# blairstar/NaturalDiffusion

Hardware: AMD Instinct MI355X
Metric: images/sec at 15-step Natural Inference (CIFAR10 32x32, NCSN++), 3-stream throughput (higher is better)
Workload: dtype bf16; 1 GPU; CIFAR10 NI 15-step step_15_weight_173.npz B=512/GPU NCSN++ 61.8M bf16, ni_step fp64 history; nfe=15, batch_per_gpu=512, streams=3

## Files before the change

### include/natinf_ncsnpp.h

```cpp
#ifndef NATINF_NCSNPP_H
#define NATINF_NCSNPP_H

#include <stdint.h>
#include "natinf.h"

#ifdef __cplusplus
extern "C" {
#endif

typedef struct natinf_ncsnpp* natinf_ncsnpp_t;

#define NATINF_NCSNPP_KEEP_ACTIVATIONS 1
#define NATINF_NCSNPP_DDPM 2

int64_t natinf_ncsnpp_param_count(void);
int64_t natinf_ncsnpp_packed_bytes(void);
int64_t natinf_ncsnpp_handle_param_count(natinf_ncsnpp_t h);
int64_t natinf_ncsnpp_handle_packed_bytes(natinf_ncsnpp_t h);
int64_t natinf_ncsnpp_workspace_bytes(natinf_ncsnpp_t h, int max_batch);

int natinf_ncsnpp_create(natinf_ncsnpp_t* out, int flags);
int natinf_ncsnpp_destroy(natinf_ncsnpp_t h);

int natinf_ncsnpp_describe(natinf_ncsnpp_t h, char* buf, int cap);
// ... 19 lines not shown
int natinf_debug_gemm_fp8(int M, int N, int K, const void* a8, const float* a_scale, const void* a_mx, const void* b8, const float* b_scale,
                          const float* bias_n, void* c, void* c_mx, int c_mode, int iters, natinf_stream_t stream);
int natinf_debug_conv_gn_up(int flags);
int natinf_debug_conv_gn_fin(float* fin_scale, float* fin_shift, const float* gamma, const float* beta, int channels_per_group, float mul);
int natinf_debug_conv_gn(int res, int B, int N, int cin, int c1, const void* x, const float* scale, const float* shift, const void* w_packed, void* w_frag,
                         const void* a1, const float* bias_n, const void* resid, float out_scale, void* out, float* gn_part, int iters,
                         natinf_stream_t stream);
#define NATINF_ATTN_BLOCK_OFF_WQKV 0
#define NATINF_ATTN_BLOCK_OFF_W3 393216
#define NATINF_ATTN_BLOCK_OFF_FOLD_WQK 524288
#define NATINF_ATTN_BLOCK_OFF_FOLD_WVO 786432
#define NATINF_ATTN_BLOCK_OFF_FOLD_CQ 1048576
#define NATINF_ATTN_BLOCK_OFF_FOLD_BO 1049600
#define NATINF_ATTN_BLOCK_OFF_WQK_PACKED 1050624
#define NATINF_ATTN_BLOCK_OFF_WVO_PACKED 1181696
#define NATINF_ATTN_BLOCK_PACKED_BYTES 1312768
#define NATINF_ATTN_BLOCK_SCRATCH_BYTES_PER_SAMPLE 393216
int natinf_debug_attn_block(int plan, int B, const void* x, int x_ld, const float* scale, const float* shift, const float* w, const float* bias,
                            void* packed, void* scratch, void* out, int o_ld, float out_scale, float* gn_part, natinf_stream_t stream);
int natinf_set_gemm_variant(int variant);
int natinf_set_gemm_epilogue(int fp32_slab);
int natinf_set_gemm_pref512(int on);
int natinf_set_gemm_half_issue(int on);
int natinf_set_gemm_round_model(int on);
int natinf_set_gemm_w128(int on);
int natinf_set_gemm_raster(int rows);
int natinf_set_fuse_gn(int on);
int natinf_set_conv_gn_wide(int mask);
int natinf_set_conv_gn_w128(int mask);
int natinf_set_conv_gn_w128_min_k(int shape, int k);
int natinf_set_conv_gn_regw(int on);
int natinf_set_fuse_up(int on);
int natinf_set_fuse_up_fold(int on);
int natinf_debug_fold_up_weights(const float* w, int N, int cin, float w_mul, float* out_f32, void* out_packed, natinf_stream_t stream);
int natinf_debug_conv_up_fold(int B, int N, int cin, const void* x, const float* scale, const float* shift, const float* w, void* w_packed, void* h_scratch,
                              const float* bias_n, const float* rowvec, float out_scale, void* out, float* gn_part, int iters, natinf_stream_t stream);
int natinf_set_fuse_head(int on);
int natinf_set_fuse_gn8(int on);
int natinf_set_fuse_gn4(int on);
int natinf_set_fuse_fin(int on);
int natinf_set_conv_gn_warm(int mask);
int natinf_set_attn256(int on);
int natinf_set_attn_proj(int on);
int natinf_set_attn_waves8(int on);
int natinf_set_attn_block(int on);
int natinf_set_attn_qkv(int on);
int natinf_set_conv_gn8_tile(int one_image);
int natinf_set_gemm_splitk(int on);
int natinf_debug_set_splitk_workspace(float* ws, int max_slices);
int natinf_debug_timestamps(void* dev_buf16);

int natinf_ncsnpp_profile(natinf_ncsnpp_t h, int enable);
int natinf_ncsnpp_profile_read(natinf_ncsnpp_t h, double* ms_by_class , int64_t* launches_by_class );

int natinf_gemm_profile(int enable);
int natinf_gemm_profile_read(char* buf, int cap);

int natinf_ncsnpp_debug_tap(natinf_ncsnpp_t h, int module_idx, float* out, int64_t capacity_elems,
                            natinf_stream_t stream);

int natinf_debug_gn_stats(const void* x, int ld, int C, int HW, int B, const float* gamma, const float* beta, float* scale, float* shift, float eps, float out_mul,
                          natinf_stream_t stream);
int natinf_debug_gn_finalize(const float* P0, int tps0, int quads0, const float* P1, int tps1, int quads1, int C, int HW, int B, const float* gamma, const float* beta,
                             float* scale, float* shift, float eps, float out_mul, natinf_stream_t stream);
int natinf_debug_gn_fold(const float* P, int tps, int quads, int fold, int B, float* out, natinf_stream_t stream);
int natinf_debug_gn_apply(const void* x, int ld, int C, int logW, int logHW, int B, const float* scale, const float* shift, void* y, void* xr, int act, int mode, int pad,
// ... 13 lines not shown
```

### naturaldiffusion_amd/_lib.py

```python
from __future__ import annotations

import ctypes as C
import os
from pathlib import Path

os.environ.setdefault("GPU_MAX_HW_QUEUES", "8")

_HERE = Path(__file__).resolve().parent
LIB_PATH = Path(os.environ.get("NATINF_LIB", _HERE / "libnatinf.so"))

if not LIB_PATH.exists():
    raise ImportError(
        f"{LIB_PATH} not found: build it with `make -C {_HERE / 'csrc'}` "
        "(or `python -c 'import __graft_entry__ as g; g.build()'`). "
        "naturaldiffusion_amd has no CPU or eager-PyTorch fallback.")

lib = C.CDLL(str(LIB_PATH))

_p, _i32, _i64, _f32, _f64 = C.c_void_p, C.c_int, C.c_int64, C.c_float, C.c_double

SIGNATURES = {
    "natinf_abi_version": (C.c_int, []),
    "natinf_strerror": (C.c_char_p, [_i32]),
    "natinf_probe": (C.c_int, []),
# ... 38 lines not shown
    "natinf_weighted_mean_f16": (C.c_int, [_p, _p, _p, _p, _i32, _f32, _i64, _p]),
    "natinf_flow_input_f16": (C.c_int, [_p, _p, _p, _f32, _f32, _i64, _p]),
    "natinf_ncsnpp_param_count": (C.c_int64, []),
    "natinf_ncsnpp_workspace_bytes": (C.c_int64, [_p, _i32]),
    "natinf_ncsnpp_packed_bytes": (C.c_int64, []),
    "natinf_ncsnpp_handle_param_count": (_i64, [_p]),
    "natinf_ncsnpp_handle_packed_bytes": (_i64, [_p]),
    "natinf_ncsnpp_create": (C.c_int, [C.POINTER(_p), _i32]),
    "natinf_ncsnpp_describe": (C.c_int, [_p, C.c_char_p, _i32]),
    "natinf_ncsnpp_destroy": (C.c_int, [_p]),
    "natinf_ncsnpp_load": (C.c_int, [_p, _p, _i64, _p, _i64, _p]),
    "natinf_ncsnpp_share": (C.c_int, [_p, _p]),
    "natinf_ncsnpp_forward": (C.c_int, [_p, _p, _p, _p, _i32, _p, _i64, _p]),
    "natinf_ncsnpp_debug_tap": (C.c_int, [_p, _i32, _p, _i64, _p]),
    "natinf_ncsnpp_describe_gemms": (C.c_int, [_p, _i32, C.c_char_p, _i32]),
    "natinf_debug_gemm": (C.c_int, [_i32, _i32, _i32, _i32, _i32, _i32, _i32, _i32, _p, _p, _p, _p, _p, _i32, _f32, _i32, _p]),
    "natinf_set_gemm_variant": (C.c_int, [_i32]),
    "natinf_debug_timestamps": (C.c_int, [_p]),
    "natinf_set_gemm_epilogue": (C.c_int, [_i32]),
    "natinf_debug_gemm_fused": (C.c_int, [_i32, _i32, _i32, _i32, _p, _p, _p, _p, _p, _p, _i32, _p, _p, _f32, _i32, _p, _i32, _p, _p, _i32, _p]),
    "natinf_set_gemm_pref512": (C.c_int, [_i32]),
    "natinf_set_gemm_half_issue": (C.c_int, [_i32]),
    "natinf_set_gemm_raster": (C.c_int, [_i32]),
    "natinf_set_gemm_round_model": (C.c_int, [_i32]),
    "natinf_set_gemm_w128": (C.c_int, [_i32]),
    "natinf_set_fuse_gn": (C.c_int, [_i32]),
    "natinf_set_conv_gn_wide": (C.c_int, [_i32]),
    "natinf_set_attn_block": (C.c_int, [_i32]),
    "natinf_set_conv_gn_w128": (C.c_int, [_i32]),
    "natinf_set_conv_gn_w128_min_k": (C.c_int, [_i32, _i32]),
    "natinf_set_conv_gn_regw": (C.c_int, [_i32]),
    "natinf_set_fuse_up": (C.c_int, [_i32]),
    "natinf_set_fuse_up_fold": (C.c_int, [_i32]),
    "natinf_debug_fold_up_weights": (C.c_int, [_p, _i32, _i32, _f32, _p, _p, _p]),
    "natinf_debug_conv_up_fold": (C.c_int, [_i32, _i32, _i32, _p, _p, _p, _p, _p, _p, _p, _p, _f32, _p, _p, _i32, _p]),
    "natinf_set_fuse_head": (C.c_int, [_i32]),
    "natinf_set_fuse_gn8": (C.c_int, [_i32]),
    "natinf_set_fuse_gn4": (C.c_int, [_i32]),
    "natinf_set_fuse_fin": (C.c_int, [_i32]),
    "natinf_set_attn_proj": (C.c_int, [_i32]),
    "natinf_set_attn_waves8": (C.c_int, [_i32]),
    "natinf_set_attn_qkv": (C.c_int, [_i32]),
    "natinf_set_conv_gn_warm": (C.c_int, [_i32]),
    "natinf_set_attn256": (C.c_int, [_i32]),
    "natinf_set_conv_gn8_tile": (C.c_int, [_i32]),
    "natinf_set_gemm_splitk": (C.c_int, [_i32]),
    "natinf_debug_set_splitk_workspace": (C.c_int, [_p, _i32]),
    "natinf_debug_set_conv_operand": (C.c_int, [_i32, _p, _i32]),
    "natinf_debug_conv_gn": (C.c_int, [_i32, _i32, _i32, _i32, _i32, _p, _p, _p, _p, _p, _p, _p, _p, _f32, _p, _p, _i32, _p]),
    "natinf_debug_conv_gn_up": (C.c_int, [_i32]),
    "natinf_debug_conv_gn_fin": (C.c_int, [_p, _p, _p, _p, _i32, _f32]),
    "natinf_debug_attn_block": (C.c_int, [_i32, _i32, _p, _i32, _p, _p, _p, _p, _p, _p, _p, _i32, _f32, _p, _p]),
    "natinf_debug_gn_stats": (C.c_int, [_p, _i32, _i32, _i32, _i32, _p, _p, _p, _p, _f32, _f32, _p]),
    "natinf_debug_gn_finalize": (C.c_int, [_p, _i32, _i32, _p, _i32, _i32, _i32, _i32, _i32, _p, _p, _p, _p, _f32, _f32, _p]),
    "natinf_debug_gn_fold": (C.c_int, [_p, _i32, _i32, _i32, _i32, _p, _p]),
    "natinf_debug_gn_apply": (C.c_int, [_p, _i32, _i32, _i32, _i32, _i32, _p, _p, _p, _p, _i32, _i32, _i32, _p]),
    "natinf_debug_head_conv": (C.c_int, [_p, _i32, _i32, _p, _p, _p, _p, _p, _p]),
    "natinf_debug_time_embed": (C.c_int, [_p, _p, _i32, _p]),
    "natinf_debug_stem_im2col": (C.c_int, [_p, _p, _i32, _p]),
    "natinf_debug_pack_conv": (C.c_int, [_p, _p, _i32, _i32, _i32, _i32, _i32, _i32, _i32, _f32, _p]),
    "natinf_debug_pack_transpose": (C.c_int, [_p, _p, _i32, _i32, _i32, _p]),
    "natinf_debug_nhwc_to_nchw": (C.c_int, [_p, _i32, _i32, _i32, _i32, _p, _p]),
    "natinf_ncsnpp_profile": (C.c_int, [_p, _i32]),
    "natinf_ncsnpp_profile_read": (C.c_int, [_p, C.POINTER(C.c_double), C.POINTER(C.c_int64)]),
    "natinf_debug_quant_fp8_rows": (C.c_int, [_p, _p, _p, _i32, _i32, _p]),
    "natinf_debug_gemm_fp8": (C.c_int, [_i32, _i32, _i32, _p, _p, _p, _p, _p, _p, _p, _p, _i32, _i32, _p]),
# ... 156 lines not shown
```

### naturaldiffusion_amd/csrc/gemm_dma.h

```cpp
#pragma once
#include "ncsnpp_kernels.h"

#ifndef NATINF_SETPRIO
#define NATINF_SETPRIO 0
#endif

namespace ncsn {

template <int WM, int WN, int TM, int TN, int AVAIL>
struct EpiCfg {
    static constexpr int CROW = WN * TN * 16 + 4;
    static constexpr int bytes(int rb) { return WM * rb * 16 * CROW * 4; }
    static constexpr int RB = bytes(TM) <= AVAIL ? TM : (bytes(TM / 2) <= AVAIL ? TM / 2 : (bytes(TM / 4) <= AVAIL ? TM / 4 : 1));
    static constexpr int SLAB_ROWS = WM * RB * 16;
    static constexpr int SLAB_BYTES = bytes(RB);
    static_assert(TM % RB == 0 && SLAB_BYTES <= AVAIL, "epilogue staging does not fit");
    static constexpr int PROW = WN * TN * 16 * 2 + 16;
    static constexpr int PACK_SLAB = WM * TM * 16 * PROW;
    static constexpr int PACK_BYTES = PACK_SLAB + WM * WN * TN * 4 * 8;
    static constexpr bool PACK_OK = PACK_BYTES <= AVAIL;
    static constexpr int NEED = PACK_OK && PACK_BYTES > SLAB_BYTES ? PACK_BYTES : SLAB_BYTES;
};

template <int WM, int WN, int TM, int TN>
struct DmaCfg {
    static constexpr int NW = WM * WN, THREADS = NW * 64;
    static constexpr int BM_ = WM * TM * 16, BN_ = WN * TN * 16;
    static constexpr int STAGE_BYTES = (BM_ + BN_) * BK * 2;
    static constexpr int PA = BM_ / 8 / NW, PB = BN_ / 8 / NW;
    using Epi = EpiCfg<WM, WN, TM, TN, 2 * STAGE_BYTES + 8192>;
    static constexpr int LDS_BYTES = Epi::NEED > 2 * STAGE_BYTES ? Epi::NEED : 2 * STAGE_BYTES;
    static_assert(BM_ % (8 * NW) == 0 && BN_ % (8 * NW) == 0, "DMA pieces must divide evenly over the waves");
};

#ifdef NATINF_DEV
#define NATINF_TS(i) do { if (g.dbg_ts && tid == 0 && blockIdx.x == 0) g.dbg_ts[i] = __builtin_amdgcn_s_memtime(); } while (0)
#else
#define NATINF_TS(i) do { } while (0)
#endif
__device__ __forceinline__ float dpp_row_sum(float v) {
    asm volatile("s_nop 4" : "+v"(v));
    v += __builtin_bit_cast(float, __builtin_amdgcn_update_dpp(0, __builtin_bit_cast(int, v), 0xB1, 0xF, 0xF, true));
    asm volatile("" : "+v"(v));
    v += __builtin_bit_cast(float, __builtin_amdgcn_update_dpp(0, __builtin_bit_cast(int, v), 0x4E, 0xF, 0xF, true));
    asm volatile("" : "+v"(v));
    v += __builtin_bit_cast(float, __builtin_amdgcn_update_dpp(0, __builtin_bit_cast(int, v), 0x141, 0xF, 0xF, true));
    asm volatile("" : "+v"(v));
    v += __builtin_bit_cast(float, __builtin_amdgcn_update_dpp(0, __builtin_bit_cast(int, v), 0x140, 0xF, 0xF, true));
    asm volatile("" : "+v"(v));
    return v;
}
typedef __bf16 bf16x4_t __attribute__((ext_vector_type(4)));
typedef float f32x2 __attribute__((ext_vector_type(2)));
template <class T> __device__ __forceinline__ __attribute__((address_space(1))) T* as_global(T* p) { return (__attribute__((address_space(1))) T*)p; }
typedef unsigned gu32x4 __attribute__((ext_vector_type(4)));
typedef float gf32x4 __attribute__((ext_vector_type(4)));
__device__ __forceinline__ uint4 gload_u4(const void* p) { const gu32x4 t = *as_global(reinterpret_cast<const gu32x4*>(p)); return make_uint4(t[0], t[1], t[2], t[3]); }
__device__ __forceinline__ float4 gload_f4(const void* p) { const gf32x4 t = *as_global(reinterpret_cast<const gf32x4*>(p)); return make_float4(t[0], t[1], t[2], t[3]); }
__device__ __forceinline__ void gstore_u4(void* p, uint4 v) { *as_global(reinterpret_cast<gu32x4*>(p)) = gu32x4{v.x, v.y, v.z, v.w}; }
template <int SW, int NSW, int RPS, int PROW, bool EDGE, int DSTEP = RPS>
struct SlabCopy {
    template <class T>
    static __device__ __forceinline__ void run(const unsigned char* src, T* dst, int64_t ld, int m, int M) {
        const uint4 v = *reinterpret_cast<const uint4*>(src + SW * RPS * PROW);
        SlabCopy<SW + 1, NSW, RPS, PROW, EDGE, DSTEP>::run(src, dst, ld, m, M);
        if (!EDGE || m + SW * RPS < M) gstore_u4(dst + (int64_t)(SW * DSTEP) * ld, v);
    }
};
template <int NSW, int RPS, int PROW, bool EDGE, int DSTEP>
struct SlabCopy<NSW, NSW, RPS, PROW, EDGE, DSTEP> {
    template <class T> static __device__ __forceinline__ void run(const unsigned char*, T*, int64_t, int, int) {}
};
template <int WM, int WN, int TM, int TN, class Cfg, int ACT, bool GN, bool RES, bool DEQ = false, bool OUT8 = false, int NSAMP = 1, bool FIN = false, bool PAIR = false, bool SCALE_ALWAYS = false, int UPW = 0>
__device__ __forceinline__ void packed_tile_epilogue(const GemmArgs& g, unsigned char* smem, f32x4 (&acc)[TM][TN],
                                                     int m0, int n0, int z, int tid, int lane, int wm, int wn)
{
    const int phase = UPW > 0 ? z : 0;
    if constexpr (UPW > 0) z = 0;
    constexpr int BN_ = WN * TN * 16, BM_ = WM * TM * 16, THREADS = WM * WN * 64, PROW = OUT8 ? BN_ + 16 : Cfg::PROW;
    static_assert(!OUT8 || (!GN && !RES && TN % 2 == 0), "fp8 output: plain column terms only");
    static_assert(!PAIR || (TN % 2 == 0 && !OUT8 && !DEQ), "interleaved n-tile pairs: bf16 output");
    static_assert(NSAMP == 1 || ((NSAMP == 2 || NSAMP == 4) && WM == 1 && TM % NSAMP == 0 && !DEQ && !OUT8), "several samples per tile: one wave row, bf16 output");
    constexpr bool ACT8 = (ACT == ACT_GELU_TANH || ACT == ACT_SILU) && !GN && TN % 2 == 0 && NSAMP == 1;
    const int r = lane & 15, q = lane >> 4;
    auto ncol = [&](int j) __attribute__((always_inline)) { return PAIR ? 32 * (j >> 1) + 8 * q + 4 * (j & 1) : 16 * j + 4 * q; };
    float dn[DEQ ? TN : 1][4], rsc[DEQ ? TM : 1], rbm[DEQ ? TM : 1];
    if constexpr (DEQ) {
#pragma unroll
        for (int j = 0; j < TN; ++j) {
            const int n = n0 + wn * TN * 16 + j * 16 + q * 4;
            float4 d = make_float4(1.f, 1.f, 1.f, 1.f);
            if (g.deq_n && n < g.N) d = *reinterpret_cast<const float4*>(g.deq_n + (int64_t)z * g.deq_n_bs + n);
// ... 964 lines not shown
```

### naturaldiffusion_amd/csrc/ncsnpp.hip

```cpp
#include <hip/hip_runtime.h>
#include <stdint.h>
#include <stdio.h>
#include <string.h>
#include <stdlib.h>
#include <functional>
#include <map>
#include <memory>
#include <string>
#include <vector>

#include "natinf_ncsnpp.h"
#include "gemm_launch.h"
#include "engine_core.h"
#include "head_conv.h"
#include "attn256.h"
#include "attn_qkv.h"
#include "attn_blk256.h"

namespace {

constexpr int NF = 128, IMG = 32, TEMB = 512, NLEVEL = 4;
constexpr int CH_MULT[NLEVEL] = {1, 2, 2, 2};
constexpr float GN_EPS = 1e-6f;
constexpr float INV_SQRT2 = 0.70710678118654752440f;
inline bool attn_at(int res) { return res == 16; }

enum Kind { K_LIN, K_CONV, K_RES, K_ATTN, K_GN, K_DOWN, K_UP };
const char* kind_name(int k) { static const char* n[] = {"lin", "conv", "res", "attn", "gn", "down", "up"}; return n[k]; }

struct Mod { int idx, kind, cin, cout, up, down, res; int64_t poff; };

enum { CLS_GEMM = 0, CLS_OTHER = 1, CLS_CONV_GN = 2, CLS_CONV_GN8 = 3, N_CLS = 4 };

int g_fuse_head = 1;
constexpr int ATTN_BLK_DEFAULT = 2;
int g_attn_blk = ATTN_BLK_DEFAULT;
int g_attn_qkv = 1;
int g_attn_w8 = 1;
int g_attn_proj = 1;
int g_fuse_gn8 = 1;
int g_fuse_fin = 3;
int g_fuse_gn4 = 1;
int g_fuse_gn = 1;
constexpr int UP_FOLD_DEFAULT = 1;
int g_fuse_up_fold = UP_FOLD_DEFAULT;
int g_fuse_up = 1;

}

struct natinf_ncsnpp : EngineCore {
    int flags = 0;
    std::vector<Mod> mods;
    std::vector<int> op_cls;
    bool prof = false;
    struct Rec { hipEvent_t a, b; int cls; };
    std::vector<Rec> recs;
    std::vector<hipEvent_t> pool;
    std::map<int, TRef> taps;
    uint64_t plan_sig = 0;
    int last_B = 0; unsigned char* last_ws = nullptr;
    std::vector<unsigned char> fin_done;
};

namespace {

bool configure_ncsnpp_kernels() {
    return hipFuncSetAttribute(reinterpret_cast<const void*>(&k_head_conv), hipFuncAttributeMaxDynamicSharedMemorySize, HeadConvCfg::LDS_BYTES) == hipSuccess &&
           hipFuncSetAttribute(reinterpret_cast<const void*>(&k_qkv256), hipFuncAttributeMaxDynamicSharedMemorySize, QKV_LDS_BYTES) == hipSuccess &&
           hipFuncSetAttribute(reinterpret_cast<const void*>(&k_attn256<false>), hipFuncAttributeMaxDynamicSharedMemorySize, A256_LDS_BYTES) == hipSuccess &&
           hipFuncSetAttribute(reinterpret_cast<const void*>(&k_attn256<true>), hipFuncAttributeMaxDynamicSharedMemorySize, A256_LDS_BYTES) == hipSuccess &&
           hipFuncSetAttribute(reinterpret_cast<const void*>(&k_attn256<true, 8>), hipFuncAttributeMaxDynamicSharedMemorySize, A256_LDS_BYTES) == hipSuccess &&
           hipFuncSetAttribute(reinterpret_cast<const void*>(&k_attn_blk256), hipFuncAttributeMaxDynamicSharedMemorySize, ABLK_LDS_BYTES) == hipSuccess &&
           hipFuncSetAttribute(reinterpret_cast<const void*>(&k_attn_blk256_v2), hipFuncAttributeMaxDynamicSharedMemorySize, ABLK2_LDS_BYTES) == hipSuccess;
}

struct AttnBlk256 {
    int plan = 0;
    int B = 0;
    const bf16* x = nullptr; int x_ld = 0;
    const float* sc = nullptr; const float* sh = nullptr;
    const bf16* wqkvf = nullptr; const float* bqk = nullptr; const float* bv = nullptr; bf16* qk = nullptr; bf16* vT = nullptr;
// ... 574 lines not shown
            pack_conv(pw0, w0, TEMB, NF, 1, NF, 0, NF); pack_conv(pw1, w1, TEMB, TEMB, 1, TEMB, 0, TEMB);
            const int64_t b0 = pack_f32(pb0, TEMB), b1 = pack_f32(pb1, TEMB);
            const int64_t dw = dense_w, db = dense_b, dout = dense_out; const int dtot = dense_total;
            op(CLS_OTHER, [=](const Ctx& c) {
                hipLaunchKernelGGL(k_time_embed, dim3(grid1d((int64_t)c.B * 128, 256, 1 << 30)), dim3(256), 0, c.stream, c.labels, c.at<bf16>(emb), c.B);
            });
            op(CLS_GEMM, [=](const Ctx& c) {
                GemmArgs g = gemm_defaults();
                g.a0 = c.at<bf16>(emb); g.a0_ld = NF; g.a0_C = NF; g.M = c.B; g.N = TEMB;
                g.b = c.w<bf16>(w0); g.b_ld = NF; g.bias_n = c.w<float>(b0); g.act = ACT_SILU;
                g.c = c.at<bf16>(t1); g.c_ld = TEMB;
                launch_gemm(g, c.stream);
                g = gemm_defaults();
                g.a0 = c.at<bf16>(t1); g.a0_ld = TEMB; g.a0_C = TEMB; g.M = c.B; g.N = TEMB;
                g.b = c.w<bf16>(w1); g.b_ld = TEMB; g.bias_n = c.w<float>(b1); g.act = ACT_SILU;
                g.c = c.at<bf16>(t2); g.c_ld = TEMB;
                launch_gemm(g, c.stream);
                g = gemm_defaults();
                g.a0 = c.at<bf16>(t2); g.a0_ld = TEMB; g.a0_C = TEMB; g.M = c.B; g.N = dtot;
                g.b = c.w<bf16>(dw); g.b_ld = TEMB; g.bias_n = c.w<float>(db);
                g.c = c.at<float>(dout); g.c_ld = dtot; g.c_mode = OUT_F32;
                launch_gemm(g, c.stream);
            });
        }
        int si = 0;
        TRef cur = skip_slot(si++);
        {
            const Mod& m = M[mi++];
            const int64_t pw = take((int64_t)NF * 27), pb = take(NF);
            const int64_t w = wres((int64_t)NF * 64 * 2);
            pack_zero(w, (int64_t)NF * 64);
            pack_conv(pw, w, NF, 3, 9, 64, 0, 3);
            const int64_t b = pack_f32(pb, NF);
            const int64_t a0 = arena.alloc((int64_t)IMG * IMG * 64 * 2);
            const TRef dst = cur;
            const Part po = register_output(dst);
            op(CLS_OTHER, [=](const Ctx& c) {
                const int64_t rows = (int64_t)c.B * IMG * IMG;
                hipLaunchKernelGGL(k_stem_im2col, dim3((unsigned)((rows * 8 + 255) / 256)), dim3(256), 0, c.stream, c.x, c.at<bf16>(a0), rows);
            });
            op(CLS_GEMM, [=](const Ctx& c) {
                const int64_t rows = (int64_t)c.B * IMG * IMG;
                GemmArgs g = gemm_defaults();
                g.a0 = c.at<bf16>(a0); g.a0_ld = 64; g.a0_C = 64; g.M = (int)rows; g.N = NF;
                g.b = c.w<bf16>(w); g.b_ld = 64; g.bias_n = c.w<float>(b);
                g.c = c.act(dst); g.c_ld = dst.ld;
                if (po.valid) { g.gn_part = c.at<float>(po.off); g.gn_quads = po.quads; }
                const int bm = launch_gemm(g, c.stream);
                if (po.valid) c.part_bm[po.id] = bm;
            });
            arena.release(a0);
            E.taps[m.idx] = dst;
        }
        int res = IMG;
        for (int l = 0; l < NLEVEL; ++l) {
            for (int b = 0; b < NUM_RES; ++b) {
                const Mod& m = M[mi++];
                const TRef dst = skip_slot(si++);
                if (attn_at(res)) {
                    TRef tmp = new_act(res, m.cout);
                    emit_res(m, cur, tmp);
                    emit_attn(M[mi++], tmp, dst);
                    arena.release(tmp.off);
                } else {
                    emit_res(m, cur, dst);
                }
                cur = dst;
            }
            if (l != NLEVEL - 1) {
                const Mod& m = M[mi++];
                const TRef dst = skip_slot(si++);
                if (ddpm) emit_downconv(m, cur, dst); else emit_res(m, cur, dst);
                cur = dst; res /= 2;
            }
        }
        {
            TRef a = new_act(res, cur.C), b = new_act(res, cur.C);
            emit_res(M[mi++], cur, a);
            emit_attn(M[mi++], a, b);
            arena.release(a.off);
            emit_res(M[mi++], b, h_slot(0));
            arena.release(b.off);
        }
        int j = 0;
// ... 93 lines not shown
const natinf_ncsnpp& reference_engine() {
    static natinf_ncsnpp* e = [] {
        int* knobs[] = {&g_fuse_gn, &g_fuse_up, &g_fuse_head, &g_fuse_gn8, &g_fuse_gn4, &g_fuse_fin, &g_attn_qkv, &g_attn_proj};
        int saved[sizeof(knobs) / sizeof(knobs[0])];
        for (size_t i = 0; i < sizeof(knobs) / sizeof(knobs[0]); ++i) { saved[i] = *knobs[i]; *knobs[i] = 1; }
        g_fuse_fin = 3;
        const int saved_fold = g_fuse_up_fold;
        g_fuse_up_fold = 0;
        natinf_ncsnpp* r = make_engine(0);
        g_fuse_up_fold = saved_fold;
        for (size_t i = 0; i < sizeof(knobs) / sizeof(knobs[0]); ++i) *knobs[i] = saved[i];
        return r;
    }();
    return *e;
}

}

extern "C" {

int64_t natinf_ncsnpp_param_count(void) { return reference_engine().n_params; }
int64_t natinf_ncsnpp_packed_bytes(void) { return reference_engine().packed_bytes; }

int64_t natinf_ncsnpp_handle_param_count(natinf_ncsnpp_t h) { return h ? h->n_params : NATINF_EINVAL; }
int64_t natinf_ncsnpp_handle_packed_bytes(natinf_ncsnpp_t h) { return h ? h->packed_bytes : NATINF_EINVAL; }

int64_t natinf_ncsnpp_workspace_bytes(natinf_ncsnpp_t h, int max_batch) {
    if (!h || max_batch <= 0) return NATINF_EINVAL;
    return h->ws_per_image * (int64_t)max_batch;
}

static uint64_t plan_signature() {
    const int k[] = {g_fuse_head, g_attn_qkv, g_attn_w8, g_attn_proj, g_fuse_gn8, g_fuse_fin, g_fuse_gn4, g_fuse_gn, g_cg_wide, g_fuse_up,
                     g_attn_blk , g_fuse_up_fold, g_cg3 };
    uint64_t h = 1469598103934665603ull;
    for (int v : k) h = (h ^ (uint64_t)(v & 0xff)) * 1099511628211ull;
    return h;
}

int natinf_ncsnpp_create(natinf_ncsnpp_t* out, int flags) {
    if (!out || (flags & ~(NATINF_NCSNPP_KEEP_ACTIVATIONS | NATINF_NCSNPP_DDPM))) return NATINF_EINVAL;
    natinf_ncsnpp* e = make_engine(flags);
    if (!e) return NATINF_ESTATE;
    e->plan_sig = plan_signature();
    *out = e;
    return NATINF_OK;
}

int natinf_ncsnpp_destroy(natinf_ncsnpp_t h) {
    if (!h) return NATINF_EINVAL;
    for (auto& r : h->recs) { (void)hipEventDestroy(r.a); (void)hipEventDestroy(r.b); }
    for (auto e : h->pool) (void)hipEventDestroy(e);
    delete h;
    return NATINF_OK;
}

int natinf_ncsnpp_describe(natinf_ncsnpp_t h, char* buf, int cap) {
    if (!h || !buf || cap <= 0) return NATINF_EINVAL;
    std::string s;
    char line[160];
    for (const auto& m : h->mods) {
        snprintf(line, sizeof(line), "%d %s %d %d %d %d %d %lld\n", m.idx, kind_name(m.kind), m.cin, m.cout, m.up, m.down, m.res,
                 (long long)m.poff);
        s += line;
    }
    if ((int)s.size() + 1 > cap) return NATINF_EINVAL;
    memcpy(buf, s.c_str(), s.size() + 1);
// ... 257 lines not shown
#ifdef NATINF_DEV
    g_dbg_ts = reinterpret_cast<unsigned long long*>(dev_buf16); return NATINF_OK;
#else
    (void)dev_buf16; return NATINF_ESTATE;
#endif
}

int natinf_set_gemm_raster(int rows) { g_raster_g = rows; return NATINF_OK; }
int natinf_set_fuse_gn(int on) { g_fuse_gn = on != 0; return NATINF_OK; }
int natinf_set_fuse_gn8(int on) { g_fuse_gn8 = on != 0; return NATINF_OK; }
int natinf_set_attn256(int on) { return on ? NATINF_OK : NATINF_ESTATE; }
int natinf_set_conv_gn_warm(int mask) { if (mask < 0 || mask > 15) return NATINF_EINVAL; g_cg_warm = mask; return NATINF_OK; }
int natinf_set_attn_block(int on) { g_attn_blk = on < 0 ? ATTN_BLK_DEFAULT : (on > 2 ? 2 : on); return NATINF_OK; }
int natinf_set_attn_qkv(int on) { g_attn_qkv = on != 0; return NATINF_OK; }
int natinf_set_attn_waves8(int on) { g_attn_w8 = on != 0; return NATINF_OK; }
int natinf_set_attn_proj(int on) { g_attn_proj = on != 0; return NATINF_OK; }
int natinf_set_fuse_fin(int on) {
    if (on < 0 || on > 3) return NATINF_EINVAL;
    static const int mask[4] = {0, 3, 1, 2};
    g_fuse_fin = mask[on];
    return NATINF_OK;
}
int natinf_set_gemm_round_model(int on) { g_round_model = on != 0; g_round_model_w128 = on >= 10 ? on : 13; return NATINF_OK; }
int natinf_set_gemm_w128(int on) { g_w128 = on < 0 ? 0 : (on > 2 ? 2 : on); return NATINF_OK; }
int natinf_set_fuse_gn4(int on) { g_fuse_gn4 = on != 0; return NATINF_OK; }
int natinf_set_conv_gn8_tile(int one_image) { return one_image ? NATINF_OK : NATINF_ESTATE; }
int natinf_set_fuse_head(int on) { g_fuse_head = on != 0; return NATINF_OK; }
int natinf_set_conv_gn_w128(int mask) { if (mask < 0 || mask > 7) return NATINF_EINVAL; g_cg3 = mask; return NATINF_OK; }
int natinf_set_conv_gn_w128_min_k(int shape, int k) { if (shape < 0 || shape > 2 || k < 0) return NATINF_EINVAL; g_cg3_min_k[shape] = k; return NATINF_OK; }
int natinf_set_conv_gn_wide(int mask) { if (mask < 0 || mask > 3) return NATINF_EINVAL; g_cg_wide = mask; return NATINF_OK; }
int natinf_set_conv_gn_regw(int on) { return on ? NATINF_OK : NATINF_ESTATE; }
int natinf_set_fuse_up(int on) { g_fuse_up = on != 0; return NATINF_OK; }
int natinf_set_fuse_up_fold(int on) { g_fuse_up_fold = on < 0 ? UP_FOLD_DEFAULT : on != 0; return NATINF_OK; }
int natinf_set_gemm_splitk(int on) { g_splitk = on != 0; return NATINF_OK; }
int natinf_debug_set_splitk_workspace(float* ws, int max_slices) { g_dbg_splitk_ws = ws; g_dbg_splitk_max = ws ? max_slices : 0; return NATINF_OK; }
int natinf_set_gemm_half_issue(int on) { return on ? NATINF_OK : NATINF_ESTATE; }
int natinf_set_gemm_pref512(int on) { g_pref_512 = on != 0; return NATINF_OK; }
int natinf_set_gemm_epilogue(int fp32_slab) { g_epi_fp32_slab = fp32_slab != 0; return NATINF_OK; }

int natinf_set_gemm_variant(int variant) {
    if (variant < 0 || variant >= V_COUNT) return NATINF_EINVAL;
    if (!variant_shipped(variant) || variant == V_CONV_GN || variant == V_FP8_256x256) return NATINF_ESTATE;
    g_force_variant = variant;
    return NATINF_OK;
}

int natinf_gemm_profile(int enable) { g_gemm_prof.on = enable != 0; return NATINF_OK; }
int natinf_gemm_profile_read(char* buf, int cap) {
    if (!buf || cap <= 0) return NATINF_EINVAL;
    std::map<std::string, std::pair<double, int64_t>> by;
    std::vector<std::string> order;
    int rc = NATINF_OK;
    for (auto& e : g_gemm_prof.ev) {
        float ms = 0.f;
        if (hipEventSynchronize(e.b) != hipSuccess || hipEventElapsedTime(&ms, e.a, e.b) != hipSuccess) { (void)hipGetLastError(); rc = NATINF_ELAUNCH; }
        else {
            auto it = by.find(e.tag);
            if (it == by.end()) { order.push_back(e.tag); it = by.emplace(e.tag, std::make_pair(0.0, (int64_t)0)).first; }
            it->second.first += ms; it->second.second += 1;
        }
        g_gemm_prof.pool.emplace_back(e.a, e.b);
    }
    g_gemm_prof.ev.clear();
    if (rc != NATINF_OK) return rc;
    std::string out;
    for (auto& t : order) {
// ... 69 lines not shown
    if (dbg_misaligned(x, 16) || dbg_misaligned(y, 16) || dbg_misaligned(xr, 16) || dbg_misaligned(scale, 16) || dbg_misaligned(shift, 16)) return NATINF_EINVAL;
    const int Hs = 1 << (logHW - logW), Hd = mode == RS_UP ? 2 * Hs : (mode == RS_DOWN ? Hs / 2 : Hs);
    const int rows_per_img = Hd + 2 * pad;
    hipLaunchKernelGGL(k_gn_apply, dim3((unsigned)((rows_per_img + GN_ROWS - 1) / GN_ROWS), (unsigned)B), dim3(256), 0, (hipStream_t)stream, (const bf16*)x, ld, C,
                       logW, logHW, scale, shift, (bf16*)y, (bf16*)xr, act, mode, pad);
    return hipGetLastError() == hipSuccess ? NATINF_OK : NATINF_ELAUNCH;
}

int natinf_debug_head_conv(const void* x, int ld, int B, const float* scale, const float* shift, const void* w16, const float* bias, float* out, natinf_stream_t stream) {
    if (!x || !scale || !shift || !w16 || !bias || !out || B < 1 || ld < HeadConvCfg::C || ld % 8) return NATINF_EINVAL;
    if (dbg_misaligned(x, 16) || dbg_misaligned(w16, 16) || dbg_misaligned(out, 16)) return NATINF_EINVAL;
    if (hipFuncSetAttribute(reinterpret_cast<const void*>(&k_head_conv), hipFuncAttributeMaxDynamicSharedMemorySize, HeadConvCfg::LDS_BYTES) != hipSuccess) {
        (void)hipGetLastError();
        return NATINF_ENODEV;
    }
    hipLaunchKernelGGL(k_head_conv, dim3((unsigned)(B * (HeadConvCfg::RES / HeadConvCfg::ROWS))), dim3(256), HeadConvCfg::LDS_BYTES, (hipStream_t)stream,
                       (const bf16*)x, ld, scale, shift, (const bf16*)w16, bias, out);
    return hipGetLastError() == hipSuccess ? NATINF_OK : NATINF_ELAUNCH;
}

int natinf_debug_time_embed(const float* labels, void* emb, int B, natinf_stream_t stream) {
    if (!labels || !emb || B < 1 || B >= (1 << 21)) return NATINF_EINVAL;
    hipLaunchKernelGGL(k_time_embed, dim3(grid1d((int64_t)B * 128, 256, 1 << 30)), dim3(256), 0, (hipStream_t)stream, labels, (bf16*)emb, B);
    return hipGetLastError() == hipSuccess ? NATINF_OK : NATINF_ELAUNCH;
}

int natinf_debug_stem_im2col(const float* x, void* A, int B, natinf_stream_t stream) {
    if (!x || !A || B < 1 || B > (1 << 17) || dbg_misaligned(A, 16)) return NATINF_EINVAL;
    const int64_t rows = (int64_t)B * 1024;
    hipLaunchKernelGGL(k_stem_im2col, dim3((unsigned)((rows * 8 + 255) / 256)), dim3(256), 0, (hipStream_t)stream, x, (bf16*)A, rows);
    return hipGetLastError() == hipSuccess ? NATINF_OK : NATINF_ELAUNCH;
}

int natinf_debug_pack_conv(const float* src, void* dst, int N, int Cin, int taps, int dst_ld, int koff, int tap_stride_c, int chunked, float wmul, natinf_stream_t stream) {
    if (!src || !dst || N < 1 || Cin < 1 || taps < 1 || koff < 0 || (chunked != 0 && chunked != 1)) return NATINF_EINVAL;
    const int64_t n = (int64_t)N * Cin * taps;
    const int64_t span = chunked ? (int64_t)((Cin + 63) / 64) * taps * 64 : (int64_t)(taps - 1) * tap_stride_c + Cin;
    if ((!chunked && tap_stride_c < Cin) || koff + span > dst_ld || n > ((int64_t)1 << 30) * 256) return NATINF_EINVAL;
    hipLaunchKernelGGL(k_pack_conv, dim3(grid1d(n, 256, 1 << 30)), dim3(256), 0, (hipStream_t)stream, src, (bf16*)dst, N, Cin, taps, dst_ld, koff, tap_stride_c, chunked, wmul);
    return hipGetLastError() == hipSuccess ? NATINF_OK : NATINF_ELAUNCH;
}

int natinf_debug_pack_transpose(const float* src, void* dst, int K, int N, int dst_ld, natinf_stream_t stream) {
    if (!src || !dst || K < 1 || N < 1 || dst_ld < K) return NATINF_EINVAL;
    hipLaunchKernelGGL(k_pack_transpose, dim3(grid1d((int64_t)K * N, 256, 1 << 30)), dim3(256), 0, (hipStream_t)stream, src, (bf16*)dst, K, N, dst_ld);
    return hipGetLastError() == hipSuccess ? NATINF_OK : NATINF_ELAUNCH;
}

int natinf_debug_nhwc_to_nchw(const void* x, int ld, int C, int HW, int B, float* out, natinf_stream_t stream) {
    if (!x || !out || B < 1 || C < 1 || HW < 1 || ld < C) return NATINF_EINVAL;
    const int64_t total = (int64_t)B * C * HW;
    if (total > ((int64_t)1 << 30) * 256) return NATINF_EINVAL;
    hipLaunchKernelGGL(k_nhwc_to_nchw_f32, dim3(grid1d(total, 256, 1 << 30)), dim3(256), 0, (hipStream_t)stream, (const bf16*)x, ld, C, HW, out, total);
    return hipGetLastError() == hipSuccess ? NATINF_OK : NATINF_ELAUNCH;
}

}
#include "dit_engine.inc"
#include "mmdit_engine.inc"
#include "vae_engine.inc"
#include "inception_engine.inc"
```

### naturaldiffusion_amd/csrc/ncsnpp_kernels.h

```cpp
#pragma once
#include <hip/hip_runtime.h>
#include <stdint.h>
#include <type_traits>

namespace ncsn {

typedef __bf16 bf16;
typedef __bf16 bf16x8 __attribute__((ext_vector_type(8)));
typedef float f32x4 __attribute__((ext_vector_type(4)));

#ifdef NATINF_ASM_PAD
#define NATINF_PAD_PRE "s_nop 7\n\ts_nop 7\n\t"
#define NATINF_PAD_POST "\n\ts_nop 7\n\ts_nop 7"
#else
#define NATINF_PAD_PRE ""
#define NATINF_PAD_POST ""
#endif

#define NATINF_M0_ASM_BEGIN _Pragma("clang diagnostic push") _Pragma("clang diagnostic ignored \"-Winline-asm\"")
#define NATINF_M0_ASM_END _Pragma("clang diagnostic pop")

__device__ __forceinline__ void lds_poison()
{
#ifdef NATINF_LDS_POISON
    typedef uint32_t poison_u4 __attribute__((ext_vector_type(4)));
    const poison_u4 v = {0x7fc07fc0u, 0x7fc07fc0u, 0x7fc07fc0u, 0x7fc07fc0u};
    for (uint32_t a = threadIdx.x * 16; a < 163840u; a += blockDim.x * 16)
        asm volatile("ds_write_b128 %0, %1" ::"v"(a), "v"(v) : "memory");
    asm volatile("s_waitcnt lgkmcnt(0)" ::: "memory");
    __syncthreads();
#endif
}

constexpr int BM = 128, BN = 128, BK = 64;
constexpr int LDS_ROW = BK;
constexpr int TILE_ELEMS = BM * LDS_ROW;
constexpr int C_ROW = BN + 4;
constexpr int GEMM_LDS_BYTES = BM * C_ROW * 4;
static_assert(4 * TILE_ELEMS * 2 <= GEMM_LDS_BYTES, "tile buffers must fit");

enum { OUT_BF16 = 0, OUT_F32 = 1, OUT_F32_NCHW = 2, OUT_FP8_MX = 3 };
enum { ACT_NONE = 0, ACT_SILU = 1, ACT_GELU_TANH = 2, ACT_RELU = 3 };

struct GemmArgs {
    const bf16* a0; int a0_ld; int a0_C;
    const bf16* a1; int a1_ld; int a1_C;
    int taps; int logW; int logHW;
    int a0_padded;
    int M, N;
    const bf16* b; int b_ld;
    int64_t a_bs, b_bs, c_bs; int batch;
    const float* bias_n; const float* bias_m;
    const float* rowvec; int rowvec_ld; int log_rows_per_sample;
    int z_samples;
    const float* gate; int gate_ld;
    const bf16* resid; int resid_ld;
    const float* resid_f32; int resid_f32_ld;
    float scale; int act;
    const float* deq_m; const float* deq_n; int64_t deq_m_bs, deq_n_bs;
    const uint8_t* a_mx; int a_mx_ld; int64_t a_mx_bs;
    uint8_t* c_mx; int c_mx_ld; int64_t c_mx_bs;
    int raster_g;
    int epi_fp32_slab;
    unsigned long long* dbg_ts;
    void* c; int c_ld; int c_mode;
// ... 686 lines not shown
```

Baseline: 3586 images/s.

## Fuse stem im2col and conv GEMM into a single direct-conv kernel

Adds a dedicated stem kernel that loads the padded fp32 input tile into LDS, builds the 3x3x3 im2col operands on the fly, and runs MFMA with bias and GroupNorm partial statistics in the epilogue. This replaces the separate im2col kernel plus generic GEMM launch, removing the bf16 im2col buffer round-trip through global memory and one launch per forward. It is enabled by default. It adds a new translation unit and shared helper header, and keeps the group-norm partial layout compatible with the existing tile choice.

```diff
diff --git a/include/natinf_ncsnpp.h b/include/natinf_ncsnpp.h
--- a/include/natinf_ncsnpp.h
+++ b/include/natinf_ncsnpp.h
@@ -75,6 +75,8 @@
 int natinf_set_conv_gn_regw(int on);
 int natinf_set_fuse_up(int on);
 int natinf_set_fuse_up_fold(int on);
+int natinf_set_fuse_stem(int on);
+int natinf_debug_stem_fused(const float* x, const void* w_packed, const float* bias, void* out, int out_ld, float* gn_part, int B, int part_rows, natinf_stream_t stream);
 int natinf_debug_fold_up_weights(const float* w, int N, int cin, float w_mul, float* out_f32, void* out_packed, natinf_stream_t stream);
 int natinf_debug_conv_up_fold(int B, int N, int cin, const void* x, const float* scale, const float* shift, const float* w, void* w_packed, void* h_scratch,
                               const float* bias_n, const float* rowvec, float out_scale, void* out, float* gn_part, int iters, natinf_stream_t stream);
diff --git a/naturaldiffusion_amd/_lib.py b/naturaldiffusion_amd/_lib.py
--- a/naturaldiffusion_amd/_lib.py
+++ b/naturaldiffusion_amd/_lib.py
@@ -94,6 +94,8 @@
     "natinf_set_conv_gn_regw": (C.c_int, [_i32]),
     "natinf_set_fuse_up": (C.c_int, [_i32]),
     "natinf_set_fuse_up_fold": (C.c_int, [_i32]),
+    "natinf_set_fuse_stem": (C.c_int, [_i32]),
+    "natinf_debug_stem_fused": (C.c_int, [_p, _p, _p, _p, _i32, _p, _i32, _i32, _p]),
     "natinf_debug_fold_up_weights": (C.c_int, [_p, _i32, _i32, _f32, _p, _p, _p]),
     "natinf_debug_conv_up_fold": (C.c_int, [_i32, _i32, _i32, _p, _p, _p, _p, _p, _p, _p, _p, _f32, _p, _p, _i32, _p]),
     "natinf_set_fuse_head": (C.c_int, [_i32]),
diff --git a/naturaldiffusion_amd/csrc/gemm_dma.h b/naturaldiffusion_amd/csrc/gemm_dma.h
--- a/naturaldiffusion_amd/csrc/gemm_dma.h
+++ b/naturaldiffusion_amd/csrc/gemm_dma.h
@@ -38,26 +38,6 @@
 #else
 #define NATINF_TS(i) do { } while (0)
 #endif
-__device__ __forceinline__ float dpp_row_sum(float v) {
-    asm volatile("s_nop 4" : "+v"(v));
-    v += __builtin_bit_cast(float, __builtin_amdgcn_update_dpp(0, __builtin_bit_cast(int, v), 0xB1, 0xF, 0xF, true));
-    asm volatile("" : "+v"(v));
-    v += __builtin_bit_cast(float, __builtin_amdgcn_update_dpp(0, __builtin_bit_cast(int, v), 0x4E, 0xF, 0xF, true));
-    asm volatile("" : "+v"(v));
-    v += __builtin_bit_cast(float, __builtin_amdgcn_update_dpp(0, __builtin_bit_cast(int, v), 0x141, 0xF, 0xF, true));
-    asm volatile("" : "+v"(v));
-    v += __builtin_bit_cast(float, __builtin_amdgcn_update_dpp(0, __builtin_bit_cast(int, v), 0x140, 0xF, 0xF, true));
-    asm volatile("" : "+v"(v));
-    return v;
-}
-typedef __bf16 bf16x4_t __attribute__((ext_vector_type(4)));
-typedef float f32x2 __attribute__((ext_vector_type(2)));
-template <class T> __device__ __forceinline__ __attribute__((address_space(1))) T* as_global(T* p) { return (__attribute__((address_space(1))) T*)p; }
-typedef unsigned gu32x4 __attribute__((ext_vector_type(4)));
-typedef float gf32x4 __attribute__((ext_vector_type(4)));
-__device__ __forceinline__ uint4 gload_u4(const void* p) { const gu32x4 t = *as_global(reinterpret_cast<const gu32x4*>(p)); return make_uint4(t[0], t[1], t[2], t[3]); }
-__device__ __forceinline__ float4 gload_f4(const void* p) { const gf32x4 t = *as_global(reinterpret_cast<const gf32x4*>(p)); return make_float4(t[0], t[1], t[2], t[3]); }
-__device__ __forceinline__ void gstore_u4(void* p, uint4 v) { *as_global(reinterpret_cast<gu32x4*>(p)) = gu32x4{v.x, v.y, v.z, v.w}; }
 template <int SW, int NSW, int RPS, int PROW, bool EDGE, int DSTEP = RPS>
 struct SlabCopy {
     template <class T>
diff --git a/naturaldiffusion_amd/csrc/kernel_common.h b/naturaldiffusion_amd/csrc/kernel_common.h
--- /dev/null
+++ b/naturaldiffusion_amd/csrc/kernel_common.h
@@ -0,0 +1,44 @@
+#pragma once
+#include <hip/hip_runtime.h>
+#include <stdint.h>
+
+namespace ncsn {
+
+typedef __bf16 bf16;
+typedef __bf16 bf16x8 __attribute__((ext_vector_type(8)));
+typedef float f32x4 __attribute__((ext_vector_type(4)));
+
+__device__ __forceinline__ void lds_poison()
+{
+#ifdef NATINF_LDS_POISON
+    typedef uint32_t poison_u4 __attribute__((ext_vector_type(4)));
+    const poison_u4 v = {0x7fc07fc0u, 0x7fc07fc0u, 0x7fc07fc0u, 0x7fc07fc0u};
+    for (uint32_t a = threadIdx.x * 16; a < 163840u; a += blockDim.x * 16)
+        asm volatile("ds_write_b128 %0, %1" ::"v"(a), "v"(v) : "memory");
+    asm volatile("s_waitcnt lgkmcnt(0)" ::: "memory");
+    __syncthreads();
+#endif
+}
+
+__device__ __forceinline__ float dpp_row_sum(float v) {
+    asm volatile("s_nop 4" : "+v"(v));
+    v += __builtin_bit_cast(float, __builtin_amdgcn_update_dpp(0, __builtin_bit_cast(int, v), 0xB1, 0xF, 0xF, true));
+    asm volatile("" : "+v"(v));
+    v += __builtin_bit_cast(float, __builtin_amdgcn_update_dpp(0, __builtin_bit_cast(int, v), 0x4E, 0xF, 0xF, true));
+    asm volatile("" : "+v"(v));
+    v += __builtin_bit_cast(float, __builtin_amdgcn_update_dpp(0, __builtin_bit_cast(int, v), 0x141, 0xF, 0xF, true));
+    asm volatile("" : "+v"(v));
+    v += __builtin_bit_cast(float, __builtin_amdgcn_update_dpp(0, __builtin_bit_cast(int, v), 0x140, 0xF, 0xF, true));
+    asm volatile("" : "+v"(v));
+    return v;
+}
+typedef __bf16 bf16x4_t __attribute__((ext_vector_type(4)));
+typedef float f32x2 __attribute__((ext_vector_type(2)));
+template <class T> __device__ __forceinline__ __attribute__((address_space(1))) T* as_global(T* p) { return (__attribute__((address_space(1))) T*)p; }
+typedef unsigned gu32x4 __attribute__((ext_vector_type(4)));
+typedef float gf32x4 __attribute__((ext_vector_type(4)));
+__device__ __forceinline__ uint4 gload_u4(const void* p) { const gu32x4 t = *as_global(reinterpret_cast<const gu32x4*>(p)); return make_uint4(t[0], t[1], t[2], t[3]); }
+__device__ __forceinline__ float4 gload_f4(const void* p) { const gf32x4 t = *as_global(reinterpret_cast<const gf32x4*>(p)); return make_float4(t[0], t[1], t[2], t[3]); }
+__device__ __forceinline__ void gstore_u4(void* p, uint4 v) { *as_global(reinterpret_cast<gu32x4*>(p)) = gu32x4{v.x, v.y, v.z, v.w}; }
+
+}
diff --git a/naturaldiffusion_amd/csrc/ncsnpp.hip b/naturaldiffusion_amd/csrc/ncsnpp.hip
--- a/naturaldiffusion_amd/csrc/ncsnpp.hip
+++ b/naturaldiffusion_amd/csrc/ncsnpp.hip
@@ -45,8 +45,12 @@
 constexpr int UP_FOLD_DEFAULT = 1;
 int g_fuse_up_fold = UP_FOLD_DEFAULT;
 int g_fuse_up = 1;
-
-}
+constexpr int FUSE_STEM_DEFAULT = 1;
+int g_fuse_stem = FUSE_STEM_DEFAULT;
+
+}
+
+namespace ncsn_small { bool launch_stem(const float* x, const void* w_packed, const float* bias, void* out, int out_ld, float* gn_part, int gn_quads, int B, int part_rows, void* stream); }
 
 struct natinf_ncsnpp : EngineCore {
     int flags = 0;
@@ -687,24 +691,37 @@
             pack_zero(w, (int64_t)NF * 64);
             pack_conv(pw, w, NF, 3, 9, 64, 0, 3);
             const int64_t b = pack_f32(pb, NF);
-            const int64_t a0 = arena.alloc((int64_t)IMG * IMG * 64 * 2);
+            const bool fused = g_fuse_stem != 0;
+            const int64_t a0 = fused ? -1 : arena.alloc((int64_t)IMG * IMG * 64 * 2);
             const TRef dst = cur;
             const Part po = register_output(dst);
-            op(CLS_OTHER, [=](const Ctx& c) {
-                const int64_t rows = (int64_t)c.B * IMG * IMG;
-                hipLaunchKernelGGL(k_stem_im2col, dim3((unsigned)((rows * 8 + 255) / 256)), dim3(256), 0, c.stream, c.x, c.at<bf16>(a0), rows);
-            });
-            op(CLS_GEMM, [=](const Ctx& c) {
-                const int64_t rows = (int64_t)c.B * IMG * IMG;
+            auto stem_gemm = [=](const Ctx& c, const bf16* a) {
                 GemmArgs g = gemm_defaults();
-                g.a0 = c.at<bf16>(a0); g.a0_ld = 64; g.a0_C = 64; g.M = (int)rows; g.N = NF;
+                g.a0 = a; g.a0_ld = 64; g.a0_C = 64; g.M = (int)((int64_t)c.B * IMG * IMG); g.N = NF;
                 g.b = c.w<bf16>(w); g.b_ld = 64; g.bias_n = c.w<float>(b);
                 g.c = c.act(dst); g.c_ld = dst.ld;
                 if (po.valid) { g.gn_part = c.at<float>(po.off); g.gn_quads = po.quads; }
-                const int bm = launch_gemm(g, c.stream);
-                if (po.valid) c.part_bm[po.id] = bm;
-            });
-            arena.release(a0);
+                return g;
+            };
+            if (fused) {
+                op(CLS_GEMM, [=](const Ctx& c) {
+                    const GemmArgs g = stem_gemm(c, c.w<bf16>(w));
+                    const int bm = g_record ? launch_gemm(g, c.stream) : variant_bm(choose_variant(g));
+                    if (!g_record && !ncsn_small::launch_stem(c.x, g.b, g.bias_n, g.c, g.c_ld, g.gn_part, g.gn_quads, c.B, bm, (void*)c.stream)) { g_launch_error = 1; return; }
+                    if (po.valid) c.part_bm[po.id] = bm;
+                });
+            } else {
+                op(CLS_OTHER, [=](const Ctx& c) {
+                    const int64_t rows = (int64_t)c.B * IMG * IMG;
+                    hipLaunchKernelGGL(k_stem_im2col, dim3((unsigned)((rows * 8 + 255) / 256)), dim3(256), 0, c.stream, c.x, c.at<bf16>(a0), rows);
+                });
+                op(CLS_GEMM, [=](const Ctx& c) {
+                    const GemmArgs g = stem_gemm(c, c.at<bf16>(a0));
+                    const int bm = launch_gemm(g, c.stream);
+                    if (po.valid) c.part_bm[po.id] = bm;
+                });
+                arena.release(a0);
+            }
             E.taps[m.idx] = dst;
         }
         int res = IMG;
@@ -864,7 +881,7 @@
 
 static uint64_t plan_signature() {
     const int k[] = {g_fuse_head, g_attn_qkv, g_attn_w8, g_attn_proj, g_fuse_gn8, g_fuse_fin, g_fuse_gn4, g_fuse_gn, g_cg_wide, g_fuse_up,
-                     g_attn_blk , g_fuse_up_fold, g_cg3 };
+                     g_attn_blk , g_fuse_up_fold, g_cg3 , g_fuse_stem};
     uint64_t h = 1469598103934665603ull;
     for (int v : k) h = (h ^ (uint64_t)(v & 0xff)) * 1099511628211ull;
     return h;
@@ -1188,6 +1205,7 @@
 int natinf_set_conv_gn_regw(int on) { return on ? NATINF_OK : NATINF_ESTATE; }
 int natinf_set_fuse_up(int on) { g_fuse_up = on != 0; return NATINF_OK; }
 int natinf_set_fuse_up_fold(int on) { g_fuse_up_fold = on < 0 ? UP_FOLD_DEFAULT : on != 0; return NATINF_OK; }
+int natinf_set_fuse_stem(int on) { g_fuse_stem = on < 0 ? FUSE_STEM_DEFAULT : on != 0; return NATINF_OK; }
 int natinf_set_gemm_splitk(int on) { g_splitk = on != 0; return NATINF_OK; }
 int natinf_debug_set_splitk_workspace(float* ws, int max_slices) { g_dbg_splitk_ws = ws; g_dbg_splitk_max = ws ? max_slices : 0; return NATINF_OK; }
 int natinf_set_gemm_half_issue(int on) { return on ? NATINF_OK : NATINF_ESTATE; }
@@ -1323,6 +1341,13 @@
     return hipGetLastError() == hipSuccess ? NATINF_OK : NATINF_ELAUNCH;
 }
 
+int natinf_debug_stem_fused(const float* x, const void* w_packed, const float* bias, void* out, int out_ld, float* gn_part, int B, int part_rows, natinf_stream_t stream) {
+    if (!x || !w_packed || !bias || !out || B < 1 || B > (1 << 17) || dbg_misaligned(w_packed, 16) || dbg_misaligned(bias, 16) || dbg_misaligned(out, 16) || dbg_misaligned(gn_part, 8))
+        return NATINF_EINVAL;
+    if (!ncsn_small::launch_stem(x, w_packed, bias, out, out_ld, gn_part, NF / 4, B, part_rows, stream)) return NATINF_EINVAL;
+    return hipGetLastError() == hipSuccess ? NATINF_OK : NATINF_ELAUNCH;
+}
+
 int natinf_debug_pack_conv(const float* src, void* dst, int N, int Cin, int taps, int dst_ld, int koff, int tap_stride_c, int chunked, float wmul, natinf_stream_t stream) {
     if (!src || !dst || N < 1 || Cin < 1 || taps < 1 || koff < 0 || (chunked != 0 && chunked != 1)) return NATINF_EINVAL;
     const int64_t n = (int64_t)N * Cin * taps;
diff --git a/naturaldiffusion_amd/csrc/ncsnpp_kernels.h b/naturaldiffusion_amd/csrc/ncsnpp_kernels.h
--- a/naturaldiffusion_amd/csrc/ncsnpp_kernels.h
+++ b/naturaldiffusion_amd/csrc/ncsnpp_kernels.h
@@ -2,12 +2,9 @@
 #include <hip/hip_runtime.h>
 #include <stdint.h>
 #include <type_traits>
+#include "kernel_common.h"
 
 namespace ncsn {
-
-typedef __bf16 bf16;
-typedef __bf16 bf16x8 __attribute__((ext_vector_type(8)));
-typedef float f32x4 __attribute__((ext_vector_type(4)));
 
 #ifdef NATINF_ASM_PAD
 #define NATINF_PAD_PRE "s_nop 7\n\ts_nop 7\n\t"
@@ -19,18 +16,6 @@
 
 #define NATINF_M0_ASM_BEGIN _Pragma("clang diagnostic push") _Pragma("clang diagnostic ignored \"-Winline-asm\"")
 #define NATINF_M0_ASM_END _Pragma("clang diagnostic pop")
-
-__device__ __forceinline__ void lds_poison()
-{
-#ifdef NATINF_LDS_POISON
-    typedef uint32_t poison_u4 __attribute__((ext_vector_type(4)));
-    const poison_u4 v = {0x7fc07fc0u, 0x7fc07fc0u, 0x7fc07fc0u, 0x7fc07fc0u};
-    for (uint32_t a = threadIdx.x * 16; a < 163840u; a += blockDim.x * 16)
-        asm volatile("ds_write_b128 %0, %1" ::"v"(a), "v"(v) : "memory");
-    asm volatile("s_waitcnt lgkmcnt(0)" ::: "memory");
-    __syncthreads();
-#endif
-}
 
 constexpr int BM = 128, BN = 128, BK = 64;
 constexpr int LDS_ROW = BK;
diff --git a/naturaldiffusion_amd/csrc/ncsnpp_small.hip b/naturaldiffusion_amd/csrc/ncsnpp_small.hip
--- /dev/null
+++ b/naturaldiffusion_amd/csrc/ncsnpp_small.hip
@@ -0,0 +1,124 @@
+#include <hip/hip_runtime.h>
+#include <stdint.h>
+
+namespace {
+#include "kernel_common.h"
+}
+using namespace ncsn;
+
+namespace {
+
+constexpr int STEM_C = 128, STEM_K = 64, STEM_WROW = STEM_K + 8;
+constexpr int STEM_PW = 34;
+
+__global__ __launch_bounds__(256, 4) void k_stem_fused(const float* __restrict__ x, const bf16* __restrict__ w, const float* __restrict__ bias, bf16* __restrict__ out, int out_ld,
+                                                    float2* __restrict__ gn_part, int gn_quads, int tm)
+{
+    __shared__ __attribute__((aligned(16))) bf16 sW[STEM_C * STEM_WROW];
+    __shared__ float2 sred[4 * (STEM_C / 4)];
+    __shared__ __attribute__((aligned(16))) float sBias[STEM_C];
+    __shared__ float sX[3 * 18 * STEM_PW];
+    lds_poison();
+    const int tid = threadIdx.x, lane = tid & 63;
+    const int wave = __builtin_amdgcn_readfirstlane(tid >> 6);
+    const int r = lane & 15, q = lane >> 4;
+    for (int c = tid; c < STEM_C * (STEM_K / 8); c += 256)
+        *reinterpret_cast<uint4*>(sW + (c >> 3) * STEM_WROW + (c & 7) * 8) = gload_u4(w + (c >> 3) * STEM_K + (c & 7) * 8);
+    if (tid < STEM_C) sBias[tid] = bias[tid] + 0.f;
+
+    const int64_t m_b = (int64_t)blockIdx.x * (64 * tm);
+    const float* img = x + (m_b >> 10) * 3072;
+    const int y0 = (int)(m_b & 1023) >> 5, prow = 2 * tm + 2;
+    for (int e = tid; e < 3 * prow * STEM_PW; e += 256) {
+        const int c = e / (prow * STEM_PW), rem = e - c * (prow * STEM_PW), ry = rem / STEM_PW, cx = rem - ry * STEM_PW;
+        const int yy = y0 - 1 + ry, xx = cx - 1;
+        sX[e] = ((unsigned)yy < 32u && (unsigned)xx < 32u) ? img[c * 1024 + yy * 32 + xx] : 0.f;
+    }
+    int koff[8];
+#pragma unroll
+    for (int t = 0; t < 8; ++t) {
+        const int k = 8 * q + t, tap = k / 3, c = k - 3 * tap;
+        koff[t] = k < 27 ? (c * prow + tap / 3) * STEM_PW + tap % 3 : -1;
+    }
+    const int p_w = wave * (16 * tm);
+    bf16* out_w = out + (m_b + p_w) * out_ld;
+    auto fetch = [&](int i, float (&v)[8]) __attribute__((always_inline)) {
+        const int p = p_w + i * 16 + r, cell = (p >> 5) * STEM_PW + (p & 31);
+#pragma unroll
+        for (int t = 0; t < 8; ++t) {
+            const float f = sX[koff[t] < 0 ? 0 : cell + koff[t]];
+            v[t] = koff[t] < 0 ? 0.f : f;
+        }
+    };
+
+    auto ncol = [&](int j) __attribute__((always_inline)) { return 32 * (j >> 1) + 8 * q + 4 * (j & 1); };
+    __syncthreads();
+    bf16x8 fb[8];
+#pragma unroll
+    for (int j = 0; j < 8; ++j) fb[j] = *reinterpret_cast<const bf16x8*>(sW + (32 * (j >> 1) + 8 * (r >> 2) + 4 * (j & 1) + (r & 3)) * STEM_WROW + 8 * q);
+    f32x2 gs2[8], gq2[8];
+#pragma unroll
+    for (int j = 0; j < 8; ++j) { gs2[j] = f32x2{0.f, 0.f}; gq2[j] = f32x2{0.f, 0.f}; }
+    bf16x8 fz;
+#pragma unroll
+    for (int t = 0; t < 8; ++t) fz[t] = (bf16)0.f;
+    float xv[8];
+    fetch(0, xv);
+
+    for (int i = 0; i < tm; ++i) {
+        asm volatile("" ::: "memory");
+        bf16x8 fa0;
+#pragma unroll
+        for (int t = 0; t < 8; ++t) fa0[t] = (bf16)xv[t];
+        if (i + 1 < tm) fetch(i + 1, xv);
+        bf16* dst = out_w + (unsigned)((i * 16 + r) * out_ld + 8 * q);
+#pragma unroll
+        for (int p = 0; p < 4; ++p) {
+            bf16x8 o;
+#pragma unroll
+            for (int h = 0; h < 2; ++h) {
+                const int j = 2 * p + h;
+                f32x4 acc = {0.f, 0.f, 0.f, 0.f};
+                acc = __builtin_amdgcn_mfma_f32_16x16x32_bf16(fb[j], fa0, acc, 0, 0, 0);
+                acc = __builtin_amdgcn_mfma_f32_16x16x32_bf16(fz, fz, acc, 0, 0, 0);
+                const float4 ct = *reinterpret_cast<const float4*>(sBias + ncol(j));
+                const float v[4] = {acc[0] + ct.x, acc[1] + ct.y, acc[2] + ct.z, acc[3] + ct.w};
+                const f32x2 lo = {v[0], v[1]}, hi = {v[2], v[3]};
+                gs2[j] += lo; gs2[j] += hi;
+                gq2[j] = __builtin_elementwise_fma(lo, lo, gq2[j]);
+                gq2[j] = __builtin_elementwise_fma(hi, hi, gq2[j]);
+#pragma unroll
+                for (int e = 0; e < 4; ++e) o[4 * h + e] = (bf16)v[e];
+            }
+            gstore_u4(dst + 32 * p, __builtin_bit_cast(uint4, o));
+        }
+    }
+    if (!gn_part) return;
+#pragma unroll
+    for (int j = 0; j < 8; ++j) {
+        const float s = dpp_row_sum(gs2[j].x + gs2[j].y), qq = dpp_row_sum(gq2[j].x + gq2[j].y);
+        if (r == 0) sred[wave * (STEM_C / 4) + (ncol(j) >> 2)] = make_float2(s, qq);
+    }
+    __syncthreads();
+    if (tid < 2 * (STEM_C / 4)) {
+        const int pt = tid >> 5, qd = tid & 31;
+        float s = 0.f, qq = 0.f;
+#pragma unroll
+        for (int wr = 0; wr < 2; ++wr) { s += sred[(2 * pt + wr) * (STEM_C / 4) + qd].x; qq += sred[(2 * pt + wr) * (STEM_C / 4) + qd].y; }
+        gn_part[((int64_t)blockIdx.x * 2 + pt) * gn_quads + qd] = make_float2(s, qq);
+    }
+}
+
+}
+
+namespace ncsn_small {
+__attribute__((visibility("hidden"))) bool launch_stem(const float* x, const void* w_packed, const float* bias, void* out, int out_ld, float* gn_part, int gn_quads, int B,
+                                                       int part_rows, void* stream) {
+    if (B <= 0 || (int64_t)B * 1024 >= ((int64_t)1 << 31) || (part_rows != 64 && part_rows != 128 && part_rows != 256) || out_ld < STEM_C || out_ld % 8 || gn_quads < STEM_C / 4)
+        return false;
+    const int tm = part_rows / 32;
+    hipLaunchKernelGGL(k_stem_fused, dim3((unsigned)((int64_t)B * 1024 / (64 * tm))), dim3(256), 0, reinterpret_cast<hipStream_t>(stream), x,
+                       reinterpret_cast<const bf16*>(w_packed), bias, reinterpret_cast<bf16*>(out), out_ld, reinterpret_cast<float2*>(gn_part), gn_quads, tm);
+    return true;
+}
+}
```

Measured after the change: 3604 images/s, median of 6. Within noise of the previous version (+0.5%).
